# sangaprabhav/HypTokenizer

Measured on AMD Instinct MI355X. Metric: merge_steps_per_sec, higher is better.
Workload: dtype bf16 prefilter + f32 canonical

## Files before the change

hyptokenizer_amd/csrc/hm_common.h:

```cpp
#pragma once
#include <hip/hip_runtime.h>
#include <hip/hip_ext.h>
#include <math.h>
#include <stdint.h>
#include <stdio.h>
#include <stdlib.h>
#include <string.h>
#include <algorithm>
#include <map>
#include <set>
#include <string>
#include <vector>

#include "../../include/hypmerge.h"
#include "hm_device_math.h"
#include "hm_scan_plan.h"
#include "hm_state.h"
#include "hm_tie_slack.h"

#pragma clang fp contract(off)

typedef float f32x16 __attribute__((ext_vector_type(16)));
typedef __bf16 bf16x8 __attribute__((ext_vector_type(8)));

// ... 93 lines not shown
};

struct HostCtl {
    uint32_t ctr[8];
    unsigned long long ctr64[4];
    ArgminRec rec;
    ArgminRec rec2[2];
    ArgminRec loop_recs[HM_LOOP_MAX_STEPS];
    uint32_t hist[HM_DIGIT_BINS];
    unsigned long long xhist[HM_EXACT_BINS];
    uint32_t head_bad;
};

struct LoopState {
    uint32_t stop;
    uint32_t steps_done;
    ArgminRec best[2];
    uint32_t tails_done;
    uint32_t pad[1];
    unsigned long long rowkey[HM_LOOP_MAX_STEPS];
};

struct hm_engine {
    int device = 0;
    int n_cu = 256;
    ScanPlanKnobs plan;
    unsigned long long* d_queue = nullptr;
    int dyn_slots = 0;
    bool dyn_queue = true;
    unsigned long long scan_tag = 0;
    std::map<const void*, int> scan_slots;
    int head = HM_SCAN_HEAD;
    int head_ring = HM_SCAN_HEAD_RING_DEFAULT;
    int64_t argmin_col_begin = 0;
    bool head_force = false;
    int64_t head_merges = 0;
    int64_t max_rows = 0, rows_alloc = 0, n = 0;
    int d1 = 0, d = 0, NG = 0, RS = 0, sign_mode = 0;
    float* img = nullptr;
    unsigned char* img16 = nullptr;
    int key_ib = HM_KEY_IB_NARROW;
    int KC = 0, RB16 = 0;
    int precision = HM_PREFILTER_AUTO;
    bool bf16_ok = true;
    uint4* ent = nullptr;
    uint4* ent2 = nullptr;
    uint4* sorted = nullptr;
    uint32_t ent_cap = 0;
    uint32_t* d_ctr = nullptr;
    uint32_t* d_rmax2 = nullptr;
    uint32_t* d_rmax2_mem = nullptr;
    unsigned long long* d_ctr64 = nullptr;
    ArgminRec* d_rec = nullptr;
    ArgminRec* d_loop_recs = nullptr;
    LoopState* d_loop = nullptr;
    int32_t* d_len = nullptr;
    bool have_len = false;
    bool force_exact = false;
    uint32_t* d_rowcnt = nullptr;
    unsigned long long* d_xhist = nullptr;
    LoopState* h_loop = nullptr;
    bool force_f32 = false;
    SearchState st;
    ScanTiming tm;
    ArgminSeed* d_seed = nullptr;
    ArgminPart* d_parts = nullptr;
// ... 331 lines not shown
```

hyptokenizer_amd/csrc/hm_engine.hip:

```cpp
#include "hm_common.h"

static thread_local std::string g_last_error;

int hm_fail(hm_engine* e, int code, const std::string& msg)
{
    g_last_error = msg;
    if (e) e->err = msg;
    return code;
}

#define HM_WIDTH(v) v,
static const int kSupportedNG[] = {HM_SCAN_NG_LIST(HM_WIDTH, HM_SCAN_WIDTHS_ALL)};
static const int kSupportedKC[] = {HM_SCAN_KC_LIST(HM_WIDTH, HM_SCAN_WIDTHS_ALL)};
#undef HM_WIDTH

static int hm_pick_kc(int d)
{
    const int need = (d + 4 + 7) / 8;
    for (int v : kSupportedKC)
        if (v >= need) return v;
    return -1;
}

static int hm_pick_ng(int d)
{
    const int need = (d + 3) / 4;
    for (int v : kSupportedNG)
        if (v >= need) return v;
    return -1;
}

extern "C" int hm_abi_version(void) { return HM_ABI_VERSION; }

#if defined(HM_TUNING)
static const char* const kKnobNames[] = {"chunk", "tail", "tail_div", "big_rows", "shape", "incr_topk", "kc_even", "phases", "ph_share0", "ph_share1", "ph_share2", "ph_share3", "ph_share4",
                                        "ph_div1", "ph_div2", "ph_div3", "ph_div4", "ph_div5", "pipeline", "pipe_fault_at", "pipeline_pairs", "dyn", "dyn_slots", "head", "head_force", "head_ring", "argmin_col_begin"};
#endif
static std::map<std::string, double> g_default_knobs;

static int hm_apply_knob(hm_engine* e, const char* name, double v)
{
    const std::string k = name ? name : "";
    if (k == "chunk") { if (!(v >= 4 && v <= 4096)) return HM_E_ARG; e->plan.chunk_f32 = e->plan.chunk_bf16 = (int)v; }
    else if (k == "tail") { if (!(v >= 0.0 && v <= 0.9)) return HM_E_ARG; e->plan.tail_fraction = v; }
    else if (k == "tail_div") { if (!(v >= 1 && v <= 16)) return HM_E_ARG; e->plan.tail_div = (int)v; }
    else if (k == "big_rows") { if (!(v >= 0)) return HM_E_ARG; e->plan.big_min_rows = (int64_t)v; }
    else if (k == "shape") { if (!(v >= -1 && v <= 4)) return HM_E_ARG; e->plan.force_shape = (int)v; }
    else if (k == "incr_topk") e->incremental_topk = v != 0.0;
    else if (k == "phases") { if (!(v >= 1 && v <= HM_SCAN_PHASES)) return HM_E_ARG; e->plan.phases = (int)v; }
    else if (k.size() == 9 && k.compare(0, 8, "ph_share") == 0 && k[8] >= '0' && k[8] < '0' + HM_SCAN_PHASES - 1) { if (!(v >= 0.0 && v <= 1.0)) return HM_E_ARG; e->plan.ph_share[k[8] - '0'] = v; }
    else if (k.size() == 7 && k.compare(0, 6, "ph_div") == 0 && k[6] >= '1' && k[6] < '0' + HM_SCAN_PHASES) { if (!(v >= 1 && v <= 64)) return HM_E_ARG; e->plan.ph_div[k[6] - '0'] = (int)v; }
    else if (k == "dyn_slots") { if (!(v >= 0 && v <= 65536)) return HM_E_ARG; e->dyn_slots = (int)v; }
    else if (k == "head") { if (!(v == 0.0 || v == (double)HM_SCAN_HEAD)) return HM_E_ARG; e->head = (int)v; }
    else if (k == "head_force") e->head_force = v != 0.0;
    else if (k == "head_ring") { if (!(v >= 0 && v < HM_SCAN_RINGS && v == (double)(int)v)) return HM_E_ARG; e->head_ring = (int)v; }
    else if (k == "argmin_col_begin") { if (!(v >= 0)) return HM_E_ARG; e->argmin_col_begin = (int64_t)v; }
    else if (k == "expect_head_bad") { if (e->h == nullptr || (e->h->head_bad != 0u) != (v != 0.0)) return HM_E_STATE; return HM_OK; }
    else if (k == "dyn") e->dyn_queue = v != 0.0;
    else if (k == "pipeline") e->pipeline = v != 0.0;
    else if (k == "pipe_fault_at") e->pipe_fault_at = (int)v;
    else if (k == "exact_search") e->force_exact = v != 0.0;
    else if (k == "pipeline_pairs") { if (!(v >= 0)) return HM_E_ARG; e->pipeline_min_pairs = (int64_t)v; }
    else if (k == "kc_even") {
        if (e->img16 != nullptr) return HM_E_STATE;
        if (v != 0.0 && (e->KC & 1)) { e->KC += 1; e->RB16 = 16 * hm_row16_chunks(e->KC); }
    }
    else return HM_E_ARG;
    e->st.disarm();
    return HM_OK;
}

extern "C" int hm_debug_set_knob(hm_engine* e, const char* name, double value)
{
    if (!e) return hm_fail(nullptr, HM_E_ARG, "hm_debug_set_knob: engine is NULL");
    const int rc = hm_apply_knob(e, name, value);
    return rc ? hm_fail(e, rc, "hm_debug_set_knob: unknown knob or value out of range") : HM_OK;
}

extern "C" int hm_debug_set_default_knob(const char* name, double value, int clear)
{
    const std::string k = name ? name : "";
    if (clear) {
        if (k.empty()) { g_default_knobs.clear(); return hm_graph_default_knob(nullptr, 0.0, 1); }
        if (hm_graph_owns_knob(name)) return hm_graph_default_knob(name, 0.0, 1);
        g_default_knobs.erase(k);
        return HM_OK;
    }
    if (const int gk = hm_graph_default_knob(name, value, 0); gk <= 0)
// ... 271 lines not shown
```

hyptokenizer_amd/csrc/hm_scan.hip:

```cpp
#include <type_traits>

#include "hm_common.h"

#pragma clang fp contract(off)


template <int CNT>
__device__ __forceinline__ void hm_dma_group(const char* src, uint32_t dst)
{
    uint32_t keep;
    if constexpr (CNT == 4)
        asm volatile("s_mov_b32 %0, m0\n\ts_mov_b32 m0, %2\n\ts_nop 0\n\tglobal_load_lds_dwordx4 %1, off\n\t"
                     "global_load_lds_dwordx4 %1, off offset:1024\n\tglobal_load_lds_dwordx4 %1, off offset:2048\n\t"
                     "global_load_lds_dwordx4 %1, off offset:3072\n\ts_mov_b32 m0, %0"
                     : "=&s"(keep) : "v"(src), "s"(dst) : "memory");
    else if constexpr (CNT == 3)
        asm volatile("s_mov_b32 %0, m0\n\ts_mov_b32 m0, %2\n\ts_nop 0\n\tglobal_load_lds_dwordx4 %1, off\n\t"
                     "global_load_lds_dwordx4 %1, off offset:1024\n\tglobal_load_lds_dwordx4 %1, off offset:2048\n\t"
                     "s_mov_b32 m0, %0"
                     : "=&s"(keep) : "v"(src), "s"(dst) : "memory");
    else if constexpr (CNT == 2)
        asm volatile("s_mov_b32 %0, m0\n\ts_mov_b32 m0, %2\n\ts_nop 0\n\tglobal_load_lds_dwordx4 %1, off\n\t"
                     "global_load_lds_dwordx4 %1, off offset:1024\n\ts_mov_b32 m0, %0"
                     : "=&s"(keep) : "v"(src), "s"(dst) : "memory");
    else
        asm volatile("s_mov_b32 %0, m0\n\ts_mov_b32 m0, %2\n\ts_nop 0\n\tglobal_load_lds_dwordx4 %1, off\n\ts_mov_b32 m0, %0"
                     : "=&s"(keep) : "v"(src), "s"(dst) : "memory");
}

template <int PIECES, int FIRST = 0>
__device__ __forceinline__ void hm_dma_run(const char* src, uint32_t dst)
{
    if constexpr (FIRST < PIECES) {
        hm_dma_group<(PIECES - FIRST < 4 ? PIECES - FIRST : 4)>(src + FIRST * 1024, dst + FIRST * 1024u);
        hm_dma_run<PIECES, FIRST + 4>(src, dst);
    }
}

#ifndef HM_SCAN_PIPE_MAX_TM
#define HM_SCAN_PIPE_MAX_TM 2
#endif
#ifndef HM_SCAN_DEEP_PREFETCH
#define HM_SCAN_DEEP_PREFETCH 1
#endif
template <int NG, int SIGN, int MODE, int BF, int TM, int WPB, int SUB, bool WK = false, int HEAD = 0, int RING = 0>
__global__ __launch_bounds__(64 * WPB, 2) void hm_scan_kernel(const ScanArgs p)
{
    static_assert(SUB % 2 == 0, "the two accumulator sets alternate between column groups: an even number per tile");
    static_assert(RING == 0 || HEAD > 0, "rings other than 0 belong to the head kernels");
    constexpr bool PIPE = (TM <= HM_SCAN_PIPE_MAX_TM);
    using G = ScanGeom<NG, BF, TM, WPB, SUB, RING>;
    constexpr int COLS = G::COLS, RS = G::RS, RB16 = G::RB16, TILE_BYTES = G::TILE_BYTES, NP = G::NP;
    constexpr int PPW = G::PPW, TILE_LDS = G::TILE_LDS, DIST = G::DIST, NBUF = G::NBUF;
    constexpr int RSUB = G::RSUB;
    static_assert(RSUB % 2 == 0, "the head walk takes the groups of a slot in pairs");
    constexpr int WAVE_ROWS = G::WAVE_ROWS, BLOCK_ROWS = G::BLOCK_ROWS, NTHREADS = G::NTHREADS;
    constexpr bool HALF_LAST = (BF != 0) && (NG & 1);
    constexpr int TCH = RS / 4 - 1;
    static_assert(HEAD == 0 || (BF != 0 && SIGN != 0 && MODE == HM_MODE_ARGMIN && PIPE && HEAD == hm_head_steps(NG)),
                  "the head test: bf16 form, lorentz sign, argmin, two accumulator sets, the head set the image's r^ was built for");
    extern __shared__ __attribute__((aligned(16))) char smem[];

    if (p.stop != nullptr && *p.stop != 0u) return;
    if (p.order_seen != nullptr && __hip_atomic_load(p.order_seen, __ATOMIC_RELAXED, __HIP_MEMORY_SCOPE_AGENT) < p.order_need) {
        if (threadIdx.x == 0) __hip_atomic_store(p.order_fault, 5u, __ATOMIC_RELAXED, __HIP_MEMORY_SCOPE_AGENT);
        return;
    }

    const int lane = threadIdx.x & 63;
    const int wave = __builtin_amdgcn_readfirstlane(threadIdx.x >> 6);
    const int r = lane & 31, h = lane >> 5;

    uint32_t sure_total = 0;
    unsigned long long gk = ~0ull;
    unsigned long long gk_raw = ~0ull;
    bool gk_pending = false;
    const uint32_t lds_base = (uint32_t)(size_t)((__attribute__((address_space(3))) char*)smem);

    uint32_t* lhist = nullptr;
    if (MODE == HM_MODE_HIST) {
        lhist = reinterpret_cast<uint32_t*>(smem + G::HIST_OFF);
        for (int t = threadIdx.x; t < HM_HIST_BINS; t += NTHREADS) lhist[t] = 0;
    }

// ... 295 lines not shown
                        const unsigned long long k = ((unsigned long long)ubz << 32) | low;
                        wkey = k < wkey ? k : wkey;
                    }
                }
                if (!emit) return;
                if (!write) { ++n_emit; return; }
                if (slot < (unsigned long long)p.ent_cap) p.ent[slot] = make_uint4(ub, (uint32_t)i, (uint32_t)j, flag);
                ++slot;
            };
#pragma unroll
            for (int e = 0; e < 16; ++e) visit(w[e], e, false);
            if (MODE == HM_MODE_HIST) continue;
            sure_total += n_sure;
            const uint32_t incl = hm_wave_incl_scan(n_emit, lane);
            const uint32_t total = __shfl(incl, 63, 64);
            if (total == 0) continue;
            unsigned long long base = 0;
            if (lane == 63) base = atomicAdd(&p.ctr64[2], (unsigned long long)total);
            base = __shfl(base, 63, 64);
            slot = base + incl - n_emit;
            asm volatile("" : "+v"(bnd), "+v"(cutv));
#pragma unroll
            for (int e = 0; e < 16; ++e) visit(w[e], e, true);
            wrote = true;
        }
        if (MODE == HM_MODE_ARGMIN && wrote) {
            const unsigned long long wk = hm_wave_min_u64(wkey);
            if (lane == 0) atomicMin(&p.ctr64[1], wk);
            gk = __hip_atomic_load(&p.ctr64[1], __ATOMIC_RELAXED, __HIP_MEMORY_SCOPE_AGENT);
            if (wk < gk) gk = wk;
        }
    };

    auto head_group = [&](auto set_c, auto red_c, int buf, int sub, bool fresh, float& ext) __attribute__((always_inline)) {
        constexpr int set = decltype(set_c)::value;
        constexpr bool RED = decltype(red_c)::value;
        constexpr int QN = 16 * TM;
        if constexpr (HEAD > 0) {
            const char* bt = smem + buf * TILE_LDS + (sub * 32 + r) * RB16 + 16 * h;
            if (fresh) {
#pragma unroll
                for (int k = 0; k < HEAD; ++k) bfr[set][k] = frag_at(bt, hm_head_kstep(k, NP));
            }
            if constexpr (RED) ext = acc[set ^ 1][0][0];
            auto kstep = [&](auto k_c) {
                constexpr int k = decltype(k_c)::value;
                constexpr int g = hm_head_kstep(k, NP);
#pragma unroll
                for (int tm = 0; tm < TM; ++tm) {
                    if constexpr (k == 0) {
                        f32x16 z;
#pragma unroll
                        for (int e = 0; e < 16; ++e) z[e] = 0.0f;
                        acc[set][tm] = mfma16(a16t[tm], bfr[set][k], z, g);
                    } else {
                        acc[set][tm] = mfma16(a16[tm][g], bfr[set][k], acc[set][tm], g);
                    }
                }
                if constexpr (RED) {
#pragma unroll
                    for (int q = (k * QN) / HEAD; q < ((k + 1) * QN) / HEAD; ++q)
                        ext = __builtin_fmaxf(ext, acc[set ^ 1][q / 16][q % 16]);
                }
            };
            kstep(std::integral_constant<int, 0>{});
            __builtin_amdgcn_sched_barrier(0);
#pragma unroll
            for (int k = 0; k < HEAD; ++k) bfr[set ^ 1][k] = frag_at(bt + 32 * RB16, hm_head_kstep(k, NP));
            __builtin_amdgcn_sched_barrier(0);
            static_assert(HEAD <= 4, "the head k-steps are written out");
            if constexpr (HEAD > 1) kstep(std::integral_constant<int, 1>{});
            if constexpr (HEAD > 2) kstep(std::integral_constant<int, 2>{});
            if constexpr (HEAD > 3) kstep(std::integral_constant<int, 3>{});
            if constexpr (RED) ext = -ext;
        }
    };
    auto head_finish = [&](auto set_c, float ext_u, int buf, int sub, int j0s) __attribute__((always_inline)) -> bool {
        constexpr int set = decltype(set_c)::value;
        if constexpr (HEAD > 0) {
            float bound_f = pre_f;
            const uint32_t best_bits = (uint32_t)(gk >> 32);
            if (best_bits != 0xffffffffu) {
                const float bb = hm::bitsf(best_bits + hm_tie_slack(best_bits)) + 2.0f * delta;
                if (bb < bound_f) bound_f = bb;
            }
            if (__ballot(ext_u < bound_f) == 0ull) return false;
            const char* bt = smem + buf * TILE_LDS + (sub * 32 + r) * RB16 + 16 * h;
            const unsigned char* as = p.img16 + (int64_t)(i0w + r) * RB16 + 16 * h;
#pragma unroll
            for (int tm = 0; tm < TM; ++tm)
#pragma unroll
                for (int e = 0; e < 16; ++e) acc[set][tm][e] = 0.0f;
#pragma unroll 1
            for (int g = 0; g < NP - 1; ++g) {
                const uint4 bv = *reinterpret_cast<const uint4*>(bt + 32 * g);
#pragma unroll
                for (int tm = 0; tm < TM; ++tm) {
                    const uint4 av = *reinterpret_cast<const uint4*>(as + (int64_t)(32 * tm) * RB16 + 32 * g);
                    acc[set][tm] = __builtin_amdgcn_mfma_f32_32x32x16_bf16(__builtin_bit_cast(bf16x8, av), __builtin_bit_cast(bf16x8, bv), acc[set][tm], 0, 0, 0);
                }
            }
            {
                const uint4 bv = frag_at(bt, NP - 1);
#pragma unroll
                for (int tm = 0; tm < TM; ++tm) {
                    uint4 av = frag_at(as + (int64_t)(32 * tm) * RB16, NP - 1);
                    if (h == 1) {
                        const uint32_t z = HALF_LAST ? av.x : av.z;
                        const uint32_t hi16 = z & 0xffffu, lo16 = z >> 16;
                        const uint32_t t0 = (hi16 | (hi16 << 16)) ^ 0x80008000u, t1 = lo16 ^ 0x8000u;
                        if (HALF_LAST) { av.x = t0; av.y = t1; }
                        else { av.z = t0; av.w = t1; }
                    }
                    acc[set][tm] = mfma16(av, bv, acc[set][tm], NP - 1);
                }
            }
            finish_group(set_c, reduce_group(set_c), j0s);
            return true;
        }
        return false;
    };

    volatile uint32_t* const qslot = reinterpret_cast<volatile uint32_t*>(smem + G::queue_off(MODE));
    const bool dyn = (MODE != HM_MODE_HIST) && (p.dyn != 0);
    unsigned long long q_raw = 0ull;
    if (dyn && threadIdx.x == 0) (void)__hip_atomic_fetch_max(p.q_ctr, p.q_tag, __ATOMIC_RELAXED, __HIP_MEMORY_SCOPE_AGENT);
    int item = (int)blockIdx.x;
#pragma unroll 1
    for (;;) {
    bool have = true;
    HM_SCAN_ITEM_DECODE(p.items, item, BLOCK_ROWS, G::PLAN_COLS, p.nct, p.col_begin, rb, ct0, ct1)
    if constexpr (COLS != G::PLAN_COLS) {
        ct0 *= G::PLAN_COLS / COLS;
        ct1 *= G::PLAN_COLS / COLS;
        if (ct0 < p.col_begin / COLS) ct0 = p.col_begin / COLS;
        if (ct1 > (p.n + COLS - 1) / COLS) ct1 = (p.n + COLS - 1) / COLS;
    }
    if (ct0 >= ct1) have = false;

    int ct_step = 1;
    if (MODE == HM_MODE_HIST && have) {
        ct_step = p.sample_stride;
        ct0 += (ct_step - (ct0 + rb * 7) % ct_step) % ct_step;
        if (ct0 >= ct1) have = false;
    }
    if (have) {
    if (rb != rb_cur) {
        rb_cur = rb;
        i0w = rb * BLOCK_ROWS + wave * WAVE_ROWS;
        wave_active = (i0w < p.row_end) && (i0w + WAVE_ROWS - 1 >= p.row_begin) && (i0w < p.n);
        rows_full = (i0w >= p.row_begin) && (i0w + WAVE_ROWS - 1 < p.row_end);
        load_a();
    }
    const int ntile = (ct1 - ct0 + ct_step - 1) / ct_step;
    auto tile_at = [&](int t) { return ct0 + t * ct_step; };

    if constexpr (RING > 0) {
#pragma unroll
        for (int q = 0; q < DIST; ++q)
            if (q < ntile) dma_tile(tile_at(q), q);
        __builtin_amdgcn_s_waitcnt(0x0F70);
    } else {
#pragma unroll
    for (int q = 0; q < DIST; ++q) dma_tile(tile_at(q < ntile ? q : ntile - 1), q);
    if (DIST - 1 <= 0) asm volatile("s_waitcnt vmcnt(0)" ::: "memory");
    else asm volatile("s_waitcnt vmcnt(%0)" ::"n"((DIST - 1) * PPW) : "memory");
    if (DIST == 1) __builtin_amdgcn_s_waitcnt(0x0F70);
    }
    __syncthreads();

    bool pend = false;
    bool deep_valid = false;
    int pend_j0s = 0;
    int buf = 0;
    int gk_due = 0;

    for (int t = 0; t < ntile; ++t) {
        const int ct = tile_at(t);
        const int ct_next = (t + DIST < ntile) ? tile_at(t + DIST) : ct;
        int buf_next = buf + DIST;
        if (buf_next >= NBUF) buf_next -= NBUF;
        const int j0 = ct * COLS;

        if (MODE == HM_MODE_ARGMIN && (t & (8 * (G::PLAN_COLS / COLS) - 1)) == 0) {
            if constexpr (RING > 0) {
                asm volatile("global_load_dwordx2 v[252:253], %0, off sc1" : : "v"(&p.ctr64[1]) : "memory", "v252", "v253");
                gk_due = t + DIST - 1;
            } else {
            asm volatile("global_load_dwordx2 %0, %1, off sc1" : "=v"(gk_raw) : "v"(&p.ctr64[1]) : "memory");
            }
            gk_pending = true;
        }
        if (dyn && t == ntile - 1 && threadIdx.x == 0) {
            if constexpr (RING > 0)
                asm volatile("global_atomic_add_x2 v[254:255], %0, %1, off sc0" : : "v"(p.q_ctr), "v"(1ull) : "memory", "v254", "v255");
            else
            asm volatile("global_atomic_add_x2 %0, %1, %2, off sc0" : "=v"(q_raw) : "v"(p.q_ctr), "v"(1ull) : "memory");
        }
        if constexpr (RING > 0) {
            if (t + DIST < ntile) dma_tile(ct_next, buf_next);
        } else {
        dma_tile(ct_next, buf_next);
        }

        if constexpr (HEAD > 0) {
            bool hp = false;
            int hg = 0, hc = 0;
#pragma unroll 1
            for (int sp = 0; sp < RSUB / 2; ++sp) {
                {
                    const int sub = 2 * sp;
                    const int j0s = j0 + sub * 32;
                    const bool do_c = wave_active && (j0s + 31 > i0w);
                    float ext_u = 0.0f;
                    if (do_c && hp) {
                        head_group(std::integral_constant<int, 0>{}, std::true_type{}, buf, sub, false, ext_u);
                    } else {
                        if (do_c) head_group(std::integral_constant<int, 0>{}, std::false_type{}, buf, sub, true, ext_u);
                        if (hp) ext_u = reduce_group(std::integral_constant<int, 1>{});
                    }
                    if (hp) { ++hg; hc += head_finish(std::integral_constant<int, 1>{}, ext_u, buf, sub - 1, j0s - 32) ? 1 : 0; }
                    hp = do_c;
                }
                {
                    const int sub = 2 * sp + 1;
                    const int j0s = j0 + sub * 32;
                    const bool do_c = wave_active && (j0s + 31 > i0w);
                    float ext_u = 0.0f;
                    if (do_c && hp) {
                        head_group(std::integral_constant<int, 1>{}, std::true_type{}, buf, sub, false, ext_u);
                    } else {
                        if (do_c) head_group(std::integral_constant<int, 1>{}, std::false_type{}, buf, sub, true, ext_u);
                        if (hp) ext_u = reduce_group(std::integral_constant<int, 0>{});
                    }
                    if (hp) { ++hg; hc += head_finish(std::integral_constant<int, 0>{}, ext_u, buf, sub - 1, j0s - 32) ? 1 : 0; }
                    hp = do_c;
                }
            }
            if (hp) { ++hg; hc += head_finish(std::integral_constant<int, 1>{}, reduce_group(std::integral_constant<int, 1>{}), buf, RSUB - 1, j0 + (RSUB - 1) * 32) ? 1 : 0; }
            hg_tot += hg; hc_tot += hc;
        } else if constexpr (!PIPE) {
            bool prev = false;
#pragma unroll 1
            for (int sub = 0; sub < SUB; ++sub) {
                const int j0s = j0 + sub * 32;
                const bool do_c = wave_active && (j0s + 31 > i0w);
                if (do_c) {
                    float ext_u = 0.0f;
                    mma_group(std::integral_constant<int, 0>{}, std::false_type{}, buf, sub, !prev, ext_u);
                    ext_u = reduce_group(std::integral_constant<int, 0>{});
                    finish_group(std::integral_constant<int, 0>{}, ext_u, j0s);
                }
                prev = do_c;
            }
        } else {
#pragma unroll 1
            for (int sp = 0; sp < SUB / 2; ++sp) {
                if constexpr (DEEP) {
                    const int ja = j0 + 2 * sp * 32, jb = ja + 32;
                    if (wave_active && (ja + 31 > i0w) && pend) {
                        float ea = 0.0f, eb = 0.0f;
                        mma_group_deep(std::integral_constant<int, 0>{}, buf, 2 * sp, !deep_valid, ea);
                        finish_group(std::integral_constant<int, 1>{}, ea, pend_j0s);
                        const bool more = 2 * sp + 2 < SUB;
                        mma_group_deep(std::integral_constant<int, 1>{}, buf, 2 * sp + 1, false, eb);
                        finish_group(std::integral_constant<int, 0>{}, eb, ja);
                        pend_j0s = jb;
                        deep_valid = more;
                        continue;
                    }
                    deep_valid = false;
                }
                {
                    const int sub = 2 * sp;
                    const int j0s = j0 + sub * 32;
                    const bool do_c = wave_active && (j0s + 31 > i0w);
                    float ext_u = 0.0f;
                    if (do_c && pend) {
                        mma_group(std::integral_constant<int, 0>{}, std::true_type{}, buf, sub, sp == 0, ext_u);
                    } else {
                        if (do_c) mma_group(std::integral_constant<int, 0>{}, std::false_type{}, buf, sub, true, ext_u);
                        if (pend) ext_u = reduce_group(std::integral_constant<int, 1>{});
                    }
                    if (pend) finish_group(std::integral_constant<int, 1>{}, ext_u, pend_j0s);
                    pend = do_c;
                    pend_j0s = j0s;
                }
                {
                    const int sub = 2 * sp + 1;
                    const int j0s = j0 + sub * 32;
                    const bool do_c = wave_active && (j0s + 31 > i0w);
                    float ext_u = 0.0f;
                    if (do_c && pend) {
                        mma_group(std::integral_constant<int, 1>{}, std::true_type{}, buf, sub, false, ext_u);
                    } else {
                        if (do_c) mma_group(std::integral_constant<int, 1>{}, std::false_type{}, buf, sub, true, ext_u);
                        if (pend) ext_u = reduce_group(std::integral_constant<int, 0>{});
                    }
                    if (pend) finish_group(std::integral_constant<int, 0>{}, ext_u, pend_j0s);
                    pend = do_c;
                    pend_j0s = j0s;
                }
            }
        }

        if constexpr (RING > 0) {
            auto ring_wait = [&](int tiles) __attribute__((always_inline)) {
                auto wait_p = [&](auto p_c) __attribute__((always_inline)) {
                    constexpr int P = decltype(p_c)::value;
                    static_assert((DIST - 1) * P <= 60, "the counted wait must fit vmcnt");
                    if (tiles >= 3 && DIST > 3) asm volatile("s_waitcnt vmcnt(%0)" : : "n"(3 * P) : "memory");
                    else if (tiles >= 2 && DIST > 2) asm volatile("s_waitcnt vmcnt(%0)" : : "n"(2 * P) : "memory");
                    else if (tiles >= 1 && DIST > 1) asm volatile("s_waitcnt vmcnt(%0)" : : "n"(P) : "memory");
                    else asm volatile("s_waitcnt vmcnt(0)" : : : "memory");
                };
                static_assert(DIST <= 4, "ring_wait writes out the depths");
                if constexpr (PREM != 0) {
                    if (wave < PREM) wait_p(std::integral_constant<int, PQ + 1>{});
                    else wait_p(std::integral_constant<int, PQ>{});
                } else {
                    wait_p(std::integral_constant<int, G::EXACT ? PQ : PPW>{});
                }
            };
            ring_wait(ntile - 2 - t);
            if (gk_pending && (t >= gk_due || t == ntile - 1)) {
                uint32_t klo, khi;
                asm volatile("v_mov_b32 %0, v252\n\tv_mov_b32 %1, v253" : "=v"(klo), "=v"(khi) : : "memory", "v252", "v253");
                gk_raw = ((unsigned long long)khi << 32) | klo;
                if (gk_raw < gk) gk = gk_raw;
                gk_pending = false;
            }
            if (dyn && t == ntile - 1 && threadIdx.x == 0) {
                uint32_t qlo, qhi;
                asm volatile("v_mov_b32 %0, v254\n\tv_mov_b32 %1, v255" : "=v"(qlo), "=v"(qhi) : : "memory", "v254", "v255");
                q_raw = ((unsigned long long)qhi << 32) | qlo;
            }
        } else {
        if (DIST - 1 <= 0) asm volatile("s_waitcnt vmcnt(0)" : "+v"(gk_raw), "+v"(q_raw) : : "memory");
        else asm volatile("s_waitcnt vmcnt(%2)" : "+v"(gk_raw), "+v"(q_raw) : "n"((DIST - 1) * PPW) : "memory");
        if (MODE == HM_MODE_ARGMIN && gk_pending) {
            if (gk_raw < gk) gk = gk_raw;
            gk_pending = false;
        }
        }
        if (dyn && t == ntile - 1 && threadIdx.x == 0) { qslot[0] = (uint32_t)q_raw; qslot[1] = (uint32_t)(q_raw >> 32); }
        __syncthreads();
        if (++buf == NBUF) buf = 0;
    }
    if constexpr (PIPE) {
        if (pend) {
            const float ext_u = reduce_group(std::integral_constant<int, 1>{});
            finish_group(std::integral_constant<int, 1>{}, ext_u, pend_j0s);
        }
    }

    if (DIST > 1 && RING == 0) { asm volatile("s_waitcnt vmcnt(0)" ::: "memory"); __syncthreads(); }
// ... 3 lines not shown
    if (!have) {
        __syncthreads();
        if (threadIdx.x == 0) {
            const unsigned long long v = __hip_atomic_fetch_add(p.q_ctr, 1ull, __ATOMIC_RELAXED, __HIP_MEMORY_SCOPE_AGENT);
            qslot[0] = (uint32_t)v; qslot[1] = (uint32_t)(v >> 32);
        }
        __syncthreads();
    }
    {
        const uint32_t qlo = __builtin_amdgcn_readfirstlane(qslot[0]), qhi = __builtin_amdgcn_readfirstlane(qslot[1]);
        const unsigned long long q = ((unsigned long long)qhi << 32) | qlo;
        if ((q >> 24) != (p.q_tag >> 24)) break;
        item = (int)gridDim.x + (int)(q & 0xffffffull);
        if (item >= p.n_items) break;
    }
    }

    if constexpr (HEAD > 0) {
        if (lane == 0 && hg_tot >= 16 && 2 * hc_tot > hg_tot) __hip_atomic_store(p.head_bad, 1u, __ATOMIC_RELAXED, __HIP_MEMORY_SCOPE_SYSTEM);
    }
    if (MODE == HM_MODE_TOPK) {
        unsigned long long s = sure_total;
#pragma unroll
        for (int off = 32; off > 0; off >>= 1) s += __shfl_xor(s, off, 64);
        if (lane == 0 && s != 0) atomicAdd(&p.ctr64[0], s);
    }
    if (MODE == HM_MODE_HIST) {
        __syncthreads();
        for (int t = threadIdx.x; t < HM_HIST_BINS; t += NTHREADS)
            if (lhist[t]) atomicAdd(&p.hist[t], lhist[t]);
    }
}

template <int NG, int SIGN, int MODE, int BF, int TM, int WPB, int SUB, bool WK = false, int HEAD = 0, int RING = 0>
static hipError_t hm_launch_scan_t(hm_engine* e, const ScanArgs& a, dim3 grid, hipStream_t s, hipEvent_t ev0, hipEvent_t ev1)
{
    using G = ScanGeom<NG, BF, TM, WPB, SUB, RING>;
    const size_t lds = G::lds_bytes(MODE);
    static_assert(RING == 0 || G::lds_bytes(MODE) <= HM_LDS_PER_BLOCK, "a deeper ring keeps two blocks per CU");
    const void* fn = reinterpret_cast<const void*>(&hm_scan_kernel<NG, SIGN, MODE, BF, TM, WPB, SUB, WK, HEAD, RING>);
    if (lds > 48 * 1024 && e->attr_done.find(fn) == e->attr_done.end()) {
        hipError_t st = hipFuncSetAttribute(fn, hipFuncAttributeMaxDynamicSharedMemorySize, (int)lds);
        if (st != hipSuccess) return st;
        e->attr_done.insert(fn);
    }
    ScanArgs b = a;
    b.n_items = (int)grid.x;
    b.dyn = 0;
    if (e->dyn_queue && MODE != HM_MODE_HIST && grid.x < (1u << 24)) {
        auto it = e->scan_slots.find(fn);
        if (it == e->scan_slots.end()) {
            int per_cu = 0;
            hipError_t st = hipOccupancyMaxActiveBlocksPerMultiprocessor(&per_cu, fn, G::NTHREADS, lds);
            if (st != hipSuccess) return st;
            it = e->scan_slots.emplace(fn, std::max(1, per_cu) * e->n_cu).first;
        }
        const int slots = e->dyn_slots > 0 ? e->dyn_slots : it->second;
        if ((int)grid.x > slots) {
            grid.x = (unsigned)slots;
            b.dyn = 1;
            b.q_tag = (++e->scan_tag) << 24;
            b.q_ctr = e->d_queue + 16 * ((b.ctr64 == e->d_ctr64) ? 0 : 1);
        }
    }
    if (ev0 != nullptr || ev1 != nullptr) hipExtLaunchKernelGGL((hm_scan_kernel<NG, SIGN, MODE, BF, TM, WPB, SUB, WK, HEAD, RING>), grid, dim3(G::NTHREADS), lds, s, ev0, ev1, 0, b);
    else hipLaunchKernelGGL((hm_scan_kernel<NG, SIGN, MODE, BF, TM, WPB, SUB, WK, HEAD, RING>), grid, dim3(G::NTHREADS), lds, s, b);
    return hipGetLastError();
}

template <int NG, int BF, int TM, int WPB, int SUB>
static hipError_t hm_launch_scan_ng(hm_engine* e, int sign, int mode, const ScanArgs& a, dim3 grid, hipStream_t s, hipEvent_t ev0,
                                    hipEvent_t ev1)
{
    if (sign) {
        if (mode == HM_MODE_TOPK) return hm_launch_scan_t<NG, 1, HM_MODE_TOPK, BF, TM, WPB, SUB>(e, a, grid, s, ev0, ev1);
        if (mode == HM_MODE_ARGMIN) {
            constexpr int HD = (BF != 0 && TM <= HM_SCAN_PIPE_MAX_TM) ? hm_head_steps(NG) : 0;
            if constexpr (HD > 0) {
                if (hm_head_live(e)) {
#define HM_HEAD_RING_CASE(R)                                                                                               \
    case R:                                                                                                                \
        if (a.key_wide) return hm_launch_scan_t<NG, 1, HM_MODE_ARGMIN, BF, TM, WPB, SUB, true, HD, R>(e, a, grid, s, ev0, ev1); \
        return hm_launch_scan_t<NG, 1, HM_MODE_ARGMIN, BF, TM, WPB, SUB, false, HD, R>(e, a, grid, s, ev0, ev1);
                    static_assert(HM_SCAN_RINGS == 3, "one case per ring");
                    switch (e->head_ring) { HM_HEAD_RING_CASE(0) HM_HEAD_RING_CASE(1) HM_HEAD_RING_CASE(2) }
#undef HM_HEAD_RING_CASE
                    return hipErrorInvalidValue;
                }
            }
            if (a.key_wide) return hm_launch_scan_t<NG, 1, HM_MODE_ARGMIN, BF, TM, WPB, SUB, true>(e, a, grid, s, ev0, ev1);
            return hm_launch_scan_t<NG, 1, HM_MODE_ARGMIN, BF, TM, WPB, SUB>(e, a, grid, s, ev0, ev1);
        }
        return hm_launch_scan_t<NG, 1, HM_MODE_HIST, BF, TM, WPB, SUB>(e, a, grid, s, ev0, ev1);
    }
    if (mode == HM_MODE_TOPK) return hm_launch_scan_t<NG, 0, HM_MODE_TOPK, BF, TM, WPB, SUB>(e, a, grid, s, ev0, ev1);
    if (mode == HM_MODE_ARGMIN) {
        if (a.key_wide) return hm_launch_scan_t<NG, 0, HM_MODE_ARGMIN, BF, TM, WPB, SUB, true>(e, a, grid, s, ev0, ev1);
        return hm_launch_scan_t<NG, 0, HM_MODE_ARGMIN, BF, TM, WPB, SUB>(e, a, grid, s, ev0, ev1);
    }
    return hm_launch_scan_t<NG, 0, HM_MODE_HIST, BF, TM, WPB, SUB>(e, a, grid, s, ev0, ev1);
}

bool hm_use_bf16(const hm_engine* e)
{
    if (!e->bf16_ok || e->force_f32) return false;
    if (e->precision == HM_PREFILTER_F32) return false;
    if (e->precision == HM_PREFILTER_BF16) return true;
    return e->d >= 24;
}

template <int S>
static hipError_t hm_launch_scan_bf16(hm_engine* e, int mode, const ScanArgs& a, dim3 grid, hipStream_t s, hipEvent_t ev0, hipEvent_t ev1)
{
    constexpr int TM = kScanShapes[S].tm, WPB = kScanShapes[S].wpb;
    static_assert(ScanGeom<13, 1, TM, WPB, HM_SUB_BF16>::BLOCK_ROWS == hm_shape_rows(S), "the item plan counts this shape's rows per block");
#define HM_KC_CASE(KCv)                                                                                                    \
    case KCv:                                                                                                              \
        if constexpr (S == 0 || KCv <= HM_SCAN_BIG_MAX_KC)                                                                 \
// ... 68 lines not shown
```

hyptokenizer_amd/csrc/hm_scan_geom.h:

```cpp
#pragma once
#include "hm_tie_slack.h"

#define HM_MAX_BLOCK_ROWS 1024
#define HM_MODE_TOPK 0
#define HM_MODE_ARGMIN 1
#define HM_MODE_HIST 2
#define HM_HIST_BINS 256

#ifndef HM_SUB_BF16
#define HM_SUB_BF16 4
#endif
#ifndef HM_SUB_F32
#define HM_SUB_F32 2
#endif
#ifndef HM_DIST_BF16
#define HM_DIST_BF16 1
#endif
#ifndef HM_SCAN_INSTANTIATE_ALL
#define HM_SCAN_INSTANTIATE_ALL 1
#endif
#ifndef HM_SCAN_ALL_SHAPES
#define HM_SCAN_ALL_SHAPES 0
#endif

HM_HOST_DEVICE_INLINE constexpr int hm_row_floats(int NG) { return 4 * NG + 4 + (((NG + 1) % 2 == 0) ? 4 : 0); }
HM_HOST_DEVICE_INLINE constexpr int hm_row16_chunks(int KC) { return KC + ((KC & 1) ? 0 : 1); }

#define HM_SCAN_NG_LIST(X, REST) REST(X(1) X(2) X(3) X(4) X(6) X(8) X(10) X(13) X(16) X(20)) X(25) REST(X(28) X(32))
#define HM_SCAN_KC_LIST(X, REST) REST(X(2) X(4) X(8)) X(13) REST(X(14) X(16))
#define HM_SCAN_WIDTHS_ALL(...) __VA_ARGS__
#if HM_SCAN_INSTANTIATE_ALL
#define HM_SCAN_WIDTHS_BUILT(...) __VA_ARGS__
#else
#define HM_SCAN_WIDTHS_BUILT(...)
#endif

struct ScanShape { int tm, wpb; };
#define HM_SCAN_SHAPES 5
constexpr ScanShape kScanShapes[HM_SCAN_SHAPES] = {{2, 4}, {4, 4}, {2, 8}, {4, 8}, {3, 4}};
#define HM_SCAN_BIG_MAX_KC 14
HM_HOST_DEVICE_INLINE constexpr int hm_shape_rows(int shape) { return 32 * kScanShapes[shape].tm * kScanShapes[shape].wpb; }
HM_HOST_DEVICE_INLINE constexpr int hm_shape_rows_max(int shape = 0)
{
    return shape == HM_SCAN_SHAPES ? 0 : (hm_shape_rows(shape) > hm_shape_rows_max(shape + 1) ? hm_shape_rows(shape) : hm_shape_rows_max(shape + 1));
}
static_assert(hm_shape_rows_max() == HM_MAX_BLOCK_ROWS, "the images are allocated with one largest block of slack rows");

struct ScanRing { int sub, dist, exact; };
#define HM_SCAN_RINGS 3
constexpr ScanRing kScanRings[HM_SCAN_RINGS] = {{0, 0, 0}, {2, 3, 0}, {2, 4, 1}};
#define HM_SCAN_HEAD_RING_DEFAULT 1
#define HM_LDS_PER_BLOCK (80 * 1024)

template <int NG, int BF, int TM, int WPB, int SUB, int RING = 0>
struct ScanGeom {
    static_assert(RING >= 0 && RING < HM_SCAN_RINGS && (RING == 0 || BF != 0), "rings other than 0: bf16 form");
    static constexpr int RSUB = kScanRings[RING].sub ? kScanRings[RING].sub : SUB;
    static constexpr bool EXACT = kScanRings[RING].exact != 0;
    static constexpr int PLAN_COLS = 32 * SUB;
    static constexpr int COLS = 32 * RSUB;
    static_assert(SUB % RSUB == 0, "an item's run of plan tiles is a whole number of ring tiles");
    static constexpr int RS = hm_row_floats(NG);
    static constexpr int RB16 = 16 * hm_row16_chunks(NG);
    static constexpr int ROW_BYTES = BF ? RB16 : RS * 4;
    static constexpr int TILE_BYTES = COLS * ROW_BYTES;
    static constexpr int NP = BF ? (NG + 1) / 2 : NG + 1;
    static constexpr int NPIECE = TILE_BYTES / 1024;
    static constexpr int PPW = (NPIECE + WPB - 1) / WPB;
    HM_HOST_DEVICE_INLINE static constexpr int wave_pieces(int w) { return EXACT ? NPIECE / WPB + (w < NPIECE % WPB ? 1 : 0) : PPW; }
    HM_HOST_DEVICE_INLINE static constexpr int wave_first(int w)
    {
        return EXACT ? w * (NPIECE / WPB) + (w < NPIECE % WPB ? w : NPIECE % WPB) : w * PPW;
    }
    static constexpr int TILE_LDS = EXACT ? TILE_BYTES : PPW * WPB * 1024;
    static constexpr int SLOTS_MAX = (HM_LDS_PER_BLOCK - 32 * ROW_BYTES - 16) / TILE_LDS;
    static constexpr int DIST = RING == 0 ? (BF ? HM_DIST_BF16 : 1)
                                          : (kScanRings[RING].dist + 1 <= SLOTS_MAX ? kScanRings[RING].dist : (SLOTS_MAX > 2 ? SLOTS_MAX - 1 : 1));
    static constexpr int NBUF = DIST + 1;
    static constexpr int WAVE_ROWS = 32 * TM;
    static constexpr int BLOCK_ROWS = WPB * WAVE_ROWS;
    static constexpr int NTHREADS = 64 * WPB;
    static_assert(TILE_BYTES % 1024 == 0, "tiles are moved in 1 KiB pieces");
    static_assert(DIST * PPW <= 60, "the counted wait must fit vmcnt");

    static constexpr int RING_BYTES = NBUF * TILE_LDS;
    static constexpr int SLACK_BYTES = 32 * ROW_BYTES;
    static constexpr int HIST_OFF = RING_BYTES;
    static constexpr int QUEUE_BYTES = 16;
    HM_HOST_DEVICE_INLINE static constexpr int queue_off(int mode)
    {
        return RING_BYTES + SLACK_BYTES + (mode == HM_MODE_HIST ? 4 * HM_HIST_BINS : 0);
    }
    HM_HOST_DEVICE_INLINE static constexpr int lds_bytes(int mode) { return queue_off(mode) + QUEUE_BYTES; }
};
```

Baseline: 5880.

## Walk head-kernel ring two tiles per barrier with a lean fused argmin path

Adds a span-2 walk for the head argmin kernels. Each iteration now processes two ring slots per __syncthreads and DMA wait, refills two slots at a time, and chains the bf16 fragment prefetch across slot boundaries. Fully right-of-diagonal tiles take a lean path that computes all four column groups and only runs the per-group finish when the wave ballot says some group beats the bound. The aim is to halve barrier and wait overhead and cut per-group branch work. In exchange the prefetch runs shallower, since fewer tiles are left in flight at each wait, and there are more template instantiations. Span 2 is the default.

```diff
diff --git a/hyptokenizer_amd/csrc/hm_common.h b/hyptokenizer_amd/csrc/hm_common.h
--- a/hyptokenizer_amd/csrc/hm_common.h
+++ b/hyptokenizer_amd/csrc/hm_common.h
@@ -149,6 +149,7 @@
     std::map<const void*, int> scan_slots;
     int head = HM_SCAN_HEAD;
     int head_ring = HM_SCAN_HEAD_RING_DEFAULT;
+    int head_span = HM_SCAN_HEAD_SPAN_DEFAULT;
     int64_t argmin_col_begin = 0;
     bool head_force = false;
     int64_t head_merges = 0;
diff --git a/hyptokenizer_amd/csrc/hm_engine.hip b/hyptokenizer_amd/csrc/hm_engine.hip
--- a/hyptokenizer_amd/csrc/hm_engine.hip
+++ b/hyptokenizer_amd/csrc/hm_engine.hip
@@ -34,7 +34,7 @@
 
 #if defined(HM_TUNING)
 static const char* const kKnobNames[] = {"chunk", "tail", "tail_div", "big_rows", "shape", "incr_topk", "kc_even", "phases", "ph_share0", "ph_share1", "ph_share2", "ph_share3", "ph_share4",
-                                        "ph_div1", "ph_div2", "ph_div3", "ph_div4", "ph_div5", "pipeline", "pipe_fault_at", "pipeline_pairs", "dyn", "dyn_slots", "head", "head_force", "head_ring", "argmin_col_begin"};
+                                        "ph_div1", "ph_div2", "ph_div3", "ph_div4", "ph_div5", "pipeline", "pipe_fault_at", "pipeline_pairs", "dyn", "dyn_slots", "head", "head_force", "head_ring", "head_span", "argmin_col_begin"};
 #endif
 static std::map<std::string, double> g_default_knobs;
 
@@ -54,6 +54,7 @@
     else if (k == "head") { if (!(v == 0.0 || v == (double)HM_SCAN_HEAD)) return HM_E_ARG; e->head = (int)v; }
     else if (k == "head_force") e->head_force = v != 0.0;
     else if (k == "head_ring") { if (!(v >= 0 && v < HM_SCAN_RINGS && v == (double)(int)v)) return HM_E_ARG; e->head_ring = (int)v; }
+    else if (k == "head_span") { if (!(v == 1.0 || v == 2.0)) return HM_E_ARG; e->head_span = (int)v; }
     else if (k == "argmin_col_begin") { if (!(v >= 0)) return HM_E_ARG; e->argmin_col_begin = (int64_t)v; }
     else if (k == "expect_head_bad") { if (e->h == nullptr || (e->h->head_bad != 0u) != (v != 0.0)) return HM_E_STATE; return HM_OK; }
     else if (k == "dyn") e->dyn_queue = v != 0.0;
diff --git a/hyptokenizer_amd/csrc/hm_scan.hip b/hyptokenizer_amd/csrc/hm_scan.hip
--- a/hyptokenizer_amd/csrc/hm_scan.hip
+++ b/hyptokenizer_amd/csrc/hm_scan.hip
@@ -43,13 +43,14 @@
 #ifndef HM_SCAN_DEEP_PREFETCH
 #define HM_SCAN_DEEP_PREFETCH 1
 #endif
-template <int NG, int SIGN, int MODE, int BF, int TM, int WPB, int SUB, bool WK = false, int HEAD = 0, int RING = 0>
+template <int NG, int SIGN, int MODE, int BF, int TM, int WPB, int SUB, bool WK = false, int HEAD = 0, int RING = 0, int SPAN = 1>
 __global__ __launch_bounds__(64 * WPB, 2) void hm_scan_kernel(const ScanArgs p)
 {
     static_assert(SUB % 2 == 0, "the two accumulator sets alternate between column groups: an even number per tile");
     static_assert(RING == 0 || HEAD > 0, "rings other than 0 belong to the head kernels");
     constexpr bool PIPE = (TM <= HM_SCAN_PIPE_MAX_TM);
-    using G = ScanGeom<NG, BF, TM, WPB, SUB, RING>;
+    using G = ScanGeom<NG, BF, TM, WPB, SUB, RING, SPAN>;
+    static_assert(G::SPAN == SPAN, "a span the ring has no slots for is the dispatch's to replace (hm_launch_scan_ng)");
     constexpr int COLS = G::COLS, RS = G::RS, RB16 = G::RB16, TILE_BYTES = G::TILE_BYTES, NP = G::NP;
     constexpr int PPW = G::PPW, TILE_LDS = G::TILE_LDS, DIST = G::DIST, NBUF = G::NBUF;
     constexpr int RSUB = G::RSUB;
@@ -411,12 +412,12 @@
         }
     };
 
-    auto head_group = [&](auto set_c, auto red_c, int buf, int sub, bool fresh, float& ext) __attribute__((always_inline)) {
+    auto head_at = [&](int buf, int sub) __attribute__((always_inline)) -> const char* { return smem + buf * TILE_LDS + (sub * 32 + r) * RB16 + 16 * h; };
+    auto head_group = [&](auto set_c, auto red_c, auto next_c, const char* bt, const char* btn, bool fresh, float& ext) __attribute__((always_inline)) {
         constexpr int set = decltype(set_c)::value;
-        constexpr bool RED = decltype(red_c)::value;
+        constexpr bool RED = decltype(red_c)::value, NEXT = decltype(next_c)::value;
         constexpr int QN = 16 * TM;
         if constexpr (HEAD > 0) {
-            const char* bt = smem + buf * TILE_LDS + (sub * 32 + r) * RB16 + 16 * h;
             if (fresh) {
 #pragma unroll
                 for (int k = 0; k < HEAD; ++k) bfr[set][k] = frag_at(bt, hm_head_kstep(k, NP));
@@ -444,8 +445,10 @@
             };
             kstep(std::integral_constant<int, 0>{});
             __builtin_amdgcn_sched_barrier(0);
-#pragma unroll
-            for (int k = 0; k < HEAD; ++k) bfr[set ^ 1][k] = frag_at(bt + 32 * RB16, hm_head_kstep(k, NP));
+            if constexpr (NEXT) {
+#pragma unroll
+                for (int k = 0; k < HEAD; ++k) bfr[set ^ 1][k] = frag_at(btn, hm_head_kstep(k, NP));
+            }
             __builtin_amdgcn_sched_barrier(0);
             static_assert(HEAD <= 4, "the head k-steps are written out");
             if constexpr (HEAD > 1) kstep(std::integral_constant<int, 1>{});
@@ -498,6 +501,95 @@
             return true;
         }
         return false;
+    };
+
+    constexpr int WMAX = ScanRun::outstanding_max(NBUF, SPAN);
+    auto ring_wait = [&](int tiles) __attribute__((always_inline)) {
+        auto wait_p = [&](auto p_c) __attribute__((always_inline)) {
+            constexpr int P = decltype(p_c)::value;
+            static_assert(WMAX * P <= 60, "the counted wait must fit vmcnt");
+            if (tiles >= 3 && WMAX >= 3) asm volatile("s_waitcnt vmcnt(%0)" : : "n"(3 * P) : "memory");
+            else if (tiles >= 2 && WMAX >= 2) asm volatile("s_waitcnt vmcnt(%0)" : : "n"(2 * P) : "memory");
+            else if (tiles >= 1 && WMAX >= 1) asm volatile("s_waitcnt vmcnt(%0)" : : "n"(P) : "memory");
+            else asm volatile("s_waitcnt vmcnt(0)" : : : "memory");
+        };
+        static_assert(RING == 0 || WMAX <= 3, "ring_wait writes out the depths");
+        if constexpr (PREM != 0) {
+            if (wave < PREM) wait_p(std::integral_constant<int, PQ + 1>{});
+            else wait_p(std::integral_constant<int, PQ>{});
+        } else {
+            wait_p(std::integral_constant<int, G::EXACT ? PQ : PPW>{});
+        }
+    };
+
+    auto head_walk = [&](int buf, int j0) __attribute__((always_inline)) {
+        if constexpr (HEAD > 0) {
+            bool hp = false;
+            int hg = 0, hc = 0;
+#pragma unroll 1
+            for (int sp = 0; sp < RSUB / 2; ++sp) {
+                {
+                    const int sub = 2 * sp;
+                    const int j0s = j0 + sub * 32;
+                    const bool do_c = wave_active && (j0s + 31 > i0w);
+                    const char* bt = head_at(buf, sub);
+                    float ext_u = 0.0f;
+                    if (do_c && hp) {
+                        head_group(std::integral_constant<int, 0>{}, std::true_type{}, std::true_type{}, bt, bt + 32 * RB16, false, ext_u);
+                    } else {
+                        if (do_c) head_group(std::integral_constant<int, 0>{}, std::false_type{}, std::true_type{}, bt, bt + 32 * RB16, true, ext_u);
+                        if (hp) ext_u = reduce_group(std::integral_constant<int, 1>{});
+                    }
+                    if (hp) { ++hg; hc += head_finish(std::integral_constant<int, 1>{}, ext_u, buf, sub - 1, j0s - 32) ? 1 : 0; }
+                    hp = do_c;
+                }
+                {
+                    const int sub = 2 * sp + 1;
+                    const int j0s = j0 + sub * 32;
+                    const bool do_c = wave_active && (j0s + 31 > i0w);
+                    const char* bt = head_at(buf, sub);
+                    float ext_u = 0.0f;
+                    if (do_c && hp) {
+                        head_group(std::integral_constant<int, 1>{}, std::true_type{}, std::true_type{}, bt, bt + 32 * RB16, false, ext_u);
+                    } else {
+                        if (do_c) head_group(std::integral_constant<int, 1>{}, std::false_type{}, std::true_type{}, bt, bt + 32 * RB16, true, ext_u);
+                        if (hp) ext_u = reduce_group(std::integral_constant<int, 0>{});
+                    }
+                    if (hp) { ++hg; hc += head_finish(std::integral_constant<int, 0>{}, ext_u, buf, sub - 1, j0s - 32) ? 1 : 0; }
+                    hp = do_c;
+                }
+            }
+            if (hp) { ++hg; hc += head_finish(std::integral_constant<int, 1>{}, reduce_group(std::integral_constant<int, 1>{}), buf, RSUB - 1, j0 + (RSUB - 1) * 32) ? 1 : 0; }
+            hg_tot += hg; hc_tot += hc;
+        }
+    };
+
+    auto head_tile_lean = [&](int buf0, int buf1, int j0) __attribute__((always_inline)) {
+        if constexpr (HEAD > 0 && SPAN == 2) {
+            static_assert(RSUB == 2, "two slots of two groups");
+            float bound_f = pre_f;
+            const uint32_t best_bits = (uint32_t)(gk >> 32);
+            if (best_bits != 0xffffffffu) {
+                const float bb = hm::bitsf(best_bits + hm_tie_slack(best_bits)) + 2.0f * delta;
+                if (bb < bound_f) bound_f = bb;
+            }
+            const char* b0 = head_at(buf0, 0);
+            const char* b1 = head_at(buf1, 0);
+            float e0 = 0.0f, e1 = 0.0f, e2 = 0.0f;
+            head_group(std::integral_constant<int, 0>{}, std::false_type{}, std::true_type{}, b0, b0 + 32 * RB16, true, e0);
+            head_group(std::integral_constant<int, 1>{}, std::true_type{}, std::true_type{}, b0 + 32 * RB16, b1, false, e0);
+            head_group(std::integral_constant<int, 0>{}, std::true_type{}, std::true_type{}, b1, b1 + 32 * RB16, false, e1);
+            head_group(std::integral_constant<int, 1>{}, std::true_type{}, std::false_type{}, b1 + 32 * RB16, b1, false, e2);
+            const float e3 = reduce_group(std::integral_constant<int, 1>{});
+            hg_tot += 2 * RSUB;
+            if (__ballot(__builtin_fminf(__builtin_fminf(e0, e1), __builtin_fminf(e2, e3)) < bound_f) != 0ull) {
+#pragma unroll 1
+                for (int g = 0; g < 2 * RSUB; ++g) {
+                    const float eg = g == 0 ? e0 : (g == 1 ? e1 : (g == 2 ? e2 : e3));
+                    hc_tot += head_finish(std::integral_constant<int, 0>{}, eg, g < RSUB ? buf0 : buf1, g % RSUB, j0 + 32 * g) ? 1 : 0;
+                }
+            }
+        }
     };
 
     volatile uint32_t* const qslot = reinterpret_cast<volatile uint32_t*>(smem + G::queue_off(MODE));
@@ -536,7 +628,7 @@
 
     if constexpr (RING > 0) {
 #pragma unroll
-        for (int q = 0; q < DIST; ++q)
+        for (int q = 0; q < NBUF - SPAN; ++q)
             if (q < ntile) dma_tile(tile_at(q), q);
         __builtin_amdgcn_s_waitcnt(0x0F70);
     } else {
@@ -554,6 +646,50 @@
     int buf = 0;
     int gk_due = 0;
 
+    if constexpr (SPAN == 2) {
+        static_assert(HEAD > 0 && RING > 0 && MODE == HM_MODE_ARGMIN, "the span-2 walk is the head kernels'");
+        const ScanRun run{ntile, NBUF, SPAN};
+        const int ntk = run.tiles();
+        const int j_right = rb * BLOCK_ROWS + BLOCK_ROWS;
+        auto ring_add = [&](int b, int q) { b += q; return b >= NBUF ? b - NBUF : b; };
+#pragma unroll 1
+        for (int k = 0; k < ntk; ++k) {
+            const int nslot = run.count(k);
+            const int j0 = (ct0 + 2 * k) * COLS;
+            const int buf1 = ring_add(buf, 1);
+            const bool last = (k == ntk - 1);
+            const bool poll = (k & 7) == 0;
+            if (poll) asm volatile("global_load_dwordx2 v[252:253], %0, off sc1" : : "v"(&p.ctr64[1]) : "memory", "v252", "v253");
+            if (dyn && last && threadIdx.x == 0)
+                asm volatile("global_atomic_add_x2 v[254:255], %0, %1, off sc0" : : "v"(p.q_ctr), "v"(1ull) : "memory", "v254", "v255");
+            {
+                const int rq = run.req_first(k), nrq = run.req_count(k);
+                const int bq = ring_add(buf, NBUF - SPAN);
+                if (nrq > 0) dma_tile(ct0 + rq, bq);
+                if (nrq > 1) dma_tile(ct0 + rq + 1, ring_add(bq, 1));
+            }
+            if (nslot == 2 && wave_active && j0 >= j_right) {
+                head_tile_lean(buf, buf1, j0);
+            } else {
+#pragma unroll 1
+                for (int sl = 0; sl < nslot; ++sl) head_walk(sl ? buf1 : buf, j0 + sl * COLS);
+            }
+            ring_wait(run.outstanding(k));
+            if (poll) {
+                uint32_t klo, khi;
+                asm volatile("v_mov_b32 %0, v252\n\tv_mov_b32 %1, v253" : "=v"(klo), "=v"(khi) : : "memory", "v252", "v253");
+                gk_raw = ((unsigned long long)khi << 32) | klo;
+                if (gk_raw < gk) gk = gk_raw;
+            }
+            if (dyn && last && threadIdx.x == 0) {
+                uint32_t qlo, qhi;
+                asm volatile("v_mov_b32 %0, v254\n\tv_mov_b32 %1, v255" : "=v"(qlo), "=v"(qhi) : : "memory", "v254", "v255");
+                qslot[0] = qlo; qslot[1] = qhi;
+            }
+            __syncthreads();
+            buf = ring_add(buf, SPAN);
+        }
+    } else
     for (int t = 0; t < ntile; ++t) {
         const int ct = tile_at(t);
         const int ct_next = (t + DIST < ntile) ? tile_at(t + DIST) : ct;
@@ -583,41 +719,7 @@
         }
 
         if constexpr (HEAD > 0) {
-            bool hp = false;
-            int hg = 0, hc = 0;
-#pragma unroll 1
-            for (int sp = 0; sp < RSUB / 2; ++sp) {
-                {
-                    const int sub = 2 * sp;
-                    const int j0s = j0 + sub * 32;
-                    const bool do_c = wave_active && (j0s + 31 > i0w);
-                    float ext_u = 0.0f;
-                    if (do_c && hp) {
-                        head_group(std::integral_constant<int, 0>{}, std::true_type{}, buf, sub, false, ext_u);
-                    } else {
-                        if (do_c) head_group(std::integral_constant<int, 0>{}, std::false_type{}, buf, sub, true, ext_u);
-                        if (hp) ext_u = reduce_group(std::integral_constant<int, 1>{});
-                    }
-                    if (hp) { ++hg; hc += head_finish(std::integral_constant<int, 1>{}, ext_u, buf, sub - 1, j0s - 32) ? 1 : 0; }
-                    hp = do_c;
-                }
-                {
-                    const int sub = 2 * sp + 1;
-                    const int j0s = j0 + sub * 32;
-                    const bool do_c = wave_active && (j0s + 31 > i0w);
-                    float ext_u = 0.0f;
-                    if (do_c && hp) {
-                        head_group(std::integral_constant<int, 1>{}, std::true_type{}, buf, sub, false, ext_u);
-                    } else {
-                        if (do_c) head_group(std::integral_constant<int, 1>{}, std::false_type{}, buf, sub, true, ext_u);
-                        if (hp) ext_u = reduce_group(std::integral_constant<int, 0>{});
-                    }
-                    if (hp) { ++hg; hc += head_finish(std::integral_constant<int, 0>{}, ext_u, buf, sub - 1, j0s - 32) ? 1 : 0; }
-                    hp = do_c;
-                }
-            }
-            if (hp) { ++hg; hc += head_finish(std::integral_constant<int, 1>{}, reduce_group(std::integral_constant<int, 1>{}), buf, RSUB - 1, j0 + (RSUB - 1) * 32) ? 1 : 0; }
-            hg_tot += hg; hc_tot += hc;
+            head_walk(buf, j0);
         } else if constexpr (!PIPE) {
             bool prev = false;
 #pragma unroll 1
@@ -684,23 +786,6 @@
         }
 
         if constexpr (RING > 0) {
-            auto ring_wait = [&](int tiles) __attribute__((always_inline)) {
-                auto wait_p = [&](auto p_c) __attribute__((always_inline)) {
-                    constexpr int P = decltype(p_c)::value;
-                    static_assert((DIST - 1) * P <= 60, "the counted wait must fit vmcnt");
-                    if (tiles >= 3 && DIST > 3) asm volatile("s_waitcnt vmcnt(%0)" : : "n"(3 * P) : "memory");
-                    else if (tiles >= 2 && DIST > 2) asm volatile("s_waitcnt vmcnt(%0)" : : "n"(2 * P) : "memory");
-                    else if (tiles >= 1 && DIST > 1) asm volatile("s_waitcnt vmcnt(%0)" : : "n"(P) : "memory");
-                    else asm volatile("s_waitcnt vmcnt(0)" : : : "memory");
-                };
-                static_assert(DIST <= 4, "ring_wait writes out the depths");
-                if constexpr (PREM != 0) {
-                    if (wave < PREM) wait_p(std::integral_constant<int, PQ + 1>{});
-                    else wait_p(std::integral_constant<int, PQ>{});
-                } else {
-                    wait_p(std::integral_constant<int, G::EXACT ? PQ : PPW>{});
-                }
-            };
             ring_wait(ntile - 2 - t);
             if (gk_pending && (t >= gk_due || t == ntile - 1)) {
                 uint32_t klo, khi;
@@ -770,13 +855,13 @@
     }
 }
 
-template <int NG, int SIGN, int MODE, int BF, int TM, int WPB, int SUB, bool WK = false, int HEAD = 0, int RING = 0>
+template <int NG, int SIGN, int MODE, int BF, int TM, int WPB, int SUB, bool WK = false, int HEAD = 0, int RING = 0, int SPAN = 1>
 static hipError_t hm_launch_scan_t(hm_engine* e, const ScanArgs& a, dim3 grid, hipStream_t s, hipEvent_t ev0, hipEvent_t ev1)
 {
-    using G = ScanGeom<NG, BF, TM, WPB, SUB, RING>;
+    using G = ScanGeom<NG, BF, TM, WPB, SUB, RING, SPAN>;
     const size_t lds = G::lds_bytes(MODE);
     static_assert(RING == 0 || G::lds_bytes(MODE) <= HM_LDS_PER_BLOCK, "a deeper ring keeps two blocks per CU");
-    const void* fn = reinterpret_cast<const void*>(&hm_scan_kernel<NG, SIGN, MODE, BF, TM, WPB, SUB, WK, HEAD, RING>);
+    const void* fn = reinterpret_cast<const void*>(&hm_scan_kernel<NG, SIGN, MODE, BF, TM, WPB, SUB, WK, HEAD, RING, SPAN>);
     if (lds > 48 * 1024 && e->attr_done.find(fn) == e->attr_done.end()) {
         hipError_t st = hipFuncSetAttribute(fn, hipFuncAttributeMaxDynamicSharedMemorySize, (int)lds);
         if (st != hipSuccess) return st;
@@ -801,8 +886,8 @@
             b.q_ctr = e->d_queue + 16 * ((b.ctr64 == e->d_ctr64) ? 0 : 1);
         }
     }
-    if (ev0 != nullptr || ev1 != nullptr) hipExtLaunchKernelGGL((hm_scan_kernel<NG, SIGN, MODE, BF, TM, WPB, SUB, WK, HEAD, RING>), grid, dim3(G::NTHREADS), lds, s, ev0, ev1, 0, b);
-    else hipLaunchKernelGGL((hm_scan_kernel<NG, SIGN, MODE, BF, TM, WPB, SUB, WK, HEAD, RING>), grid, dim3(G::NTHREADS), lds, s, b);
+    if (ev0 != nullptr || ev1 != nullptr) hipExtLaunchKernelGGL((hm_scan_kernel<NG, SIGN, MODE, BF, TM, WPB, SUB, WK, HEAD, RING, SPAN>), grid, dim3(G::NTHREADS), lds, s, ev0, ev1, 0, b);
+    else hipLaunchKernelGGL((hm_scan_kernel<NG, SIGN, MODE, BF, TM, WPB, SUB, WK, HEAD, RING, SPAN>), grid, dim3(G::NTHREADS), lds, s, b);
     return hipGetLastError();
 }
 
@@ -816,12 +901,16 @@
             constexpr int HD = (BF != 0 && TM <= HM_SCAN_PIPE_MAX_TM) ? hm_head_steps(NG) : 0;
             if constexpr (HD > 0) {
                 if (hm_head_live(e)) {
-#define HM_HEAD_RING_CASE(R)                                                                                               \
-    case R:                                                                                                                \
-        if (a.key_wide) return hm_launch_scan_t<NG, 1, HM_MODE_ARGMIN, BF, TM, WPB, SUB, true, HD, R>(e, a, grid, s, ev0, ev1); \
-        return hm_launch_scan_t<NG, 1, HM_MODE_ARGMIN, BF, TM, WPB, SUB, false, HD, R>(e, a, grid, s, ev0, ev1);
-                    static_assert(HM_SCAN_RINGS == 3, "one case per ring");
-                    switch (e->head_ring) { HM_HEAD_RING_CASE(0) HM_HEAD_RING_CASE(1) HM_HEAD_RING_CASE(2) }
+#define HM_HEAD_RING_CASE(R, S)                                                                                            \
+    case 4 * S + R: {                                                                                                      \
+        constexpr int SP = ScanGeom<NG, BF, TM, WPB, SUB, R, S>::SPAN;                                                     \
+        if (a.key_wide) return hm_launch_scan_t<NG, 1, HM_MODE_ARGMIN, BF, TM, WPB, SUB, true, HD, R, SP>(e, a, grid, s, ev0, ev1); \
+        return hm_launch_scan_t<NG, 1, HM_MODE_ARGMIN, BF, TM, WPB, SUB, false, HD, R, SP>(e, a, grid, s, ev0, ev1);       \
+    }
+                    static_assert(HM_SCAN_RINGS == 3, "one case per ring and span");
+                    switch (4 * (e->head_ring == 0 ? 1 : e->head_span) + e->head_ring) {
+                        HM_HEAD_RING_CASE(0, 1) HM_HEAD_RING_CASE(1, 1) HM_HEAD_RING_CASE(2, 1) HM_HEAD_RING_CASE(1, 2) HM_HEAD_RING_CASE(2, 2)
+                    }
 #undef HM_HEAD_RING_CASE
                     return hipErrorInvalidValue;
                 }
diff --git a/hyptokenizer_amd/csrc/hm_scan_geom.h b/hyptokenizer_amd/csrc/hm_scan_geom.h
--- a/hyptokenizer_amd/csrc/hm_scan_geom.h
+++ b/hyptokenizer_amd/csrc/hm_scan_geom.h
@@ -50,9 +50,23 @@
 #define HM_SCAN_RINGS 3
 constexpr ScanRing kScanRings[HM_SCAN_RINGS] = {{0, 0, 0}, {2, 3, 0}, {2, 4, 1}};
 #define HM_SCAN_HEAD_RING_DEFAULT 1
+#define HM_SCAN_HEAD_SPAN_DEFAULT 2
 #define HM_LDS_PER_BLOCK (80 * 1024)
 
-template <int NG, int BF, int TM, int WPB, int SUB, int RING = 0>
+struct ScanRun {
+    int ntile, nbuf, span;
+    HM_HOST_DEVICE_INLINE constexpr int clamp(int s) const { return s < 0 ? 0 : (s > ntile ? ntile : s); }
+    HM_HOST_DEVICE_INLINE constexpr int tiles() const { return (ntile + span - 1) / span; }
+    HM_HOST_DEVICE_INLINE constexpr int prologue() const { return clamp(nbuf - span); }
+    HM_HOST_DEVICE_INLINE constexpr int first(int k) const { return k * span; }
+    HM_HOST_DEVICE_INLINE constexpr int count(int k) const { return clamp((k + 1) * span) - clamp(k * span); }
+    HM_HOST_DEVICE_INLINE constexpr int req_first(int k) const { return clamp(nbuf + (k - 1) * span); }
+    HM_HOST_DEVICE_INLINE constexpr int req_count(int k) const { return clamp(nbuf + k * span) - req_first(k); }
+    HM_HOST_DEVICE_INLINE constexpr int outstanding(int k) const { return clamp(nbuf + k * span) - clamp((k + 2) * span); }
+    HM_HOST_DEVICE_INLINE static constexpr int outstanding_max(int nbuf, int span) { return nbuf - 2 * span; }
+};
+
+template <int NG, int BF, int TM, int WPB, int SUB, int RING = 0, int SPAN_ASK = 1>
 struct ScanGeom {
     static_assert(RING >= 0 && RING < HM_SCAN_RINGS && (RING == 0 || BF != 0), "rings other than 0: bf16 form");
     static constexpr int RSUB = kScanRings[RING].sub ? kScanRings[RING].sub : SUB;
@@ -77,11 +91,15 @@
     static constexpr int DIST = RING == 0 ? (BF ? HM_DIST_BF16 : 1)
                                           : (kScanRings[RING].dist + 1 <= SLOTS_MAX ? kScanRings[RING].dist : (SLOTS_MAX > 2 ? SLOTS_MAX - 1 : 1));
     static constexpr int NBUF = DIST + 1;
+    static_assert(SPAN_ASK == 1 || SPAN_ASK == 2, "the walks that are written out");
+    static constexpr int SPAN = (RING != 0 && NBUF >= 2 * SPAN_ASK) ? SPAN_ASK : 1;
+    static_assert(SPAN == 1 || NBUF >= 2 * SPAN, "a compute tile's slots and the next one's are in the ring together");
     static constexpr int WAVE_ROWS = 32 * TM;
     static constexpr int BLOCK_ROWS = WPB * WAVE_ROWS;
     static constexpr int NTHREADS = 64 * WPB;
     static_assert(TILE_BYTES % 1024 == 0, "tiles are moved in 1 KiB pieces");
     static_assert(DIST * PPW <= 60, "the counted wait must fit vmcnt");
+    static_assert(SPAN == 1 || ScanRun::outstanding_max(NBUF, SPAN) <= DIST - SPAN, "a span's waits leave less in flight than span 1's");
 
     static constexpr int RING_BYTES = NBUF * TILE_LDS;
     static constexpr int SLACK_BYTES = 32 * ROW_BYTES;
```

Result: faster. 7123, median of 6 (+21.1%).
